# uc-vision/smart-tree

Measured on AMD Instinct MI355X. Metric: points/sec end-to-end (voxelize->sparse-UNet->skeleton), 1M-pt tree, higher is better.
Workload: dtype f32

## Files before the change

### smart_tree_amd/csrc/prims.hip

```cpp
#include <cstdarg>

#include "st_common.h"

static thread_local char g_err[512] = "";

void st_set_error(const char* fmt, ...) {
    va_list ap;
    va_start(ap, fmt);
    vsnprintf(g_err, sizeof(g_err), fmt, ap);
    va_end(ap);
}

extern "C" const char* st_last_error(void) { return g_err; }
void st_stream_wait(hipStream_t stream) { (void)hipStreamSynchronize(stream); }

extern "C" int st_version(void) { return 104; }

#define SCAN_BLOCK 256
#define SCAN_ITEMS 16
#define SCAN_TILE (SCAN_BLOCK * SCAN_ITEMS)
#define SCAN_DIRECT_BLOCKS 1024

__device__ __forceinline__ void scan_load(const uint32_t* in, int64_t base, int64_t n, uint32_t (&v)[SCAN_ITEMS]) {
    if (base + SCAN_ITEMS <= n && ((((uintptr_t)in) & 15) == 0)) {
        const uint4* p = reinterpret_cast<const uint4*>(in + base);
#pragma unroll
        for (int q = 0; q < SCAN_ITEMS / 4; q++) {
            const uint4 t = p[q];
            v[4 * q] = t.x; v[4 * q + 1] = t.y; v[4 * q + 2] = t.z; v[4 * q + 3] = t.w;
        }
    } else {
// ... 261 lines not shown
```

### smart_tree_amd/csrc/skeleton.hip

```cpp
#include "st_common.h"
#include "st_grid.h"
#include "smarttree_hip.h"

#include <atomic>

#define SK_MAX_WAVES 16
#define SK_EMPTY64 0xffffffffffffffffull
#define SK_WIDE_BLOCK 256
#define SK_SSSP_BLOCKS 2048
#define SK_MARK 0xfffffffeu
#define SK_ANC 64

struct SkJob {
    unsigned seq, done, quit;
    int len, id, csz, nrows, ny, x0, y0, z0, z1, path_off;
    float rp;
    unsigned gone;
    unsigned alive;
};

struct SkArgs {
    int C;
    int64_t m;
    const int* comp_off;
    const int* comp_seg;
    int* comp_of;
    const float* pts;
    const float* rad;
    const float* ysurf;
    const uint32_t* row_off;
    const uint32_t* col;
    const float* wgt;
    const StGrid* grid;
    const uint32_t* cell_start;
// ... 8 lines not shown
    int* n_branches;
    int* path_verts;
    int* branch_of;
    unsigned* dist_ord;
    unsigned* stamp;
    unsigned* q0;
    unsigned* q1;
    unsigned* term_bits;
    unsigned* help_bits;
    float4* pr;
    unsigned long long* best;
    unsigned* touched;
    int* anc;
    unsigned* cnt;
    unsigned* fcnt;
    unsigned fseg;
    int* s_done;
    int* s_len;
    int* s_cur_id;
    int* s_cur_off;
    int* s_nb;
    int* s_total;
    float* s_rp;
    unsigned* s_ntouched;
    int* s_cursor;
    int* s_wide;
    const unsigned* order;
    const float* order_init;
    const int* blk_comp;
    const int* blk_first;
// ... 40 lines not shown
__device__ __forceinline__ float sk_dist(const float* a, const float* b) {
    const float dx = a[0] - b[0], dy = a[1] - b[1], dz = a[2] - b[2];
    float s = dx * dx;
    float t = dy * dy;
    s = s + t;
    t = dz * dz;
    s = s + t;
    return s;
}

#define SK_VERTEX_LOOP(v) \
    for (int64_t v = (int64_t)blockIdx.x * blockDim.x + threadIdx.x; v < A.m; v += (int64_t)gridDim.x * blockDim.x)

#define SK_FS 16
#define SK_Q_HOLE 0xffffffffu
__device__ __forceinline__ unsigned sk_q_reserve(unsigned* q, unsigned* fc, unsigned seg, unsigned shard, unsigned n) {
    const unsigned at = atomicAdd(&fc[shard], n);
    if (at + n <= seg) return shard * seg + at;
    for (unsigned i = at; i < seg; i++) q[shard * seg + i] = SK_Q_HOLE;
    return SK_FS * seg + atomicAdd(&fc[SK_FS], n);
}

__device__ __forceinline__ unsigned sk_q_reserve_coop(unsigned* q, unsigned* fc, unsigned seg, unsigned shard, unsigned n) {
    const unsigned at = atomicAdd(&fc[shard], n);
    if (at + n <= seg) return shard * seg + at;
    for (unsigned i = at; i < seg; i++) __hip_atomic_store(&q[shard * seg + i], SK_Q_HOLE, __ATOMIC_RELAXED, __HIP_MEMORY_SCOPE_AGENT);
    return SK_FS * seg + atomicAdd(&fc[SK_FS], n);
}

__global__ void __launch_bounds__(SK_WIDE_BLOCK) k_sk_init(SkArgs A) {
    const unsigned inf = st_f2ord(__uint_as_float(0x7f800000u));
    SK_VERTEX_LOOP(v) { A.dist_ord[v] = inf; A.stamp[v] = 0u; }
    if (blockIdx.x == 0 && threadIdx.x < 8) A.cnt[threadIdx.x] = 0u;
    if (blockIdx.x == 0)
        for (int i = threadIdx.x; i < 3 * (SK_FS + 1); i += blockDim.x) A.fcnt[i] = i == SK_FS ? (unsigned)A.C : 0u;
}

__global__ void __launch_bounds__(1024) k_sk_roots(SkArgs A) {
    __shared__ unsigned long long s_red[SK_MAX_WAVES];
    const int c = blockIdx.x, base = A.comp_off[c], n = A.comp_off[c + 1] - base;
    unsigned long long key = 0;
    for (int v = threadIdx.x; v < n; v += blockDim.x) {
        A.comp_of[base + v] = c;
        const unsigned long long k = ((unsigned long long)(0xffffffffu - st_f2ord(A.ysurf[base + v])) << 32) | (0xffffffffu - (unsigned)v);
        key = k > key ? k : key;
    }
    key = block_max_u64(key, s_red);
    if (threadIdx.x == 0) {
// ... 38 lines not shown
    const unsigned round = (unsigned)r + 1u;
    const int lane = threadIdx.x & (glanes - 1);
    const unsigned wave = threadIdx.x / glanes, nwv = blockDim.x / glanes;
    const unsigned gw = blockIdx.x * nwv + wave, tw = gridDim.x * nwv;
#define SK_RELAX(u, du, out, out_n)                                                                        \
    {                                                                                                      \
        const uint32_t s_ = A.row_off[u], e_ = A.row_off[(u) + 1];                                         \
        for (uint32_t t = s_ + lane; t < e_; t += glanes) {                                                    \
            const unsigned v = A.col[t];                                                                   \
            const unsigned o = st_f2ord((du) + A.wgt[t]);                                                  \
            if (lookfirst && o >= A.dist_ord[v]) continue;  \
            const unsigned old = atomicMin(&A.dist_ord[v], o);                                             \
            if (o < old) {                                                                                 \
                const unsigned slot = atomicAdd(out_n, 1u);                                                \
                if (slot < SK_LQ) (out)[slot] = v;                                                         \
                else if (atomicExch(&A.stamp[v], round) != round) qn[sk_q_reserve(qn, fc_out, seg, shard, 1u)] = v; \
            }                                                                                              \
        }                                                                                                  \
    }
    for (unsigned f = gw; f < count; f += tw) {
        int sh = 0;
#pragma unroll
        for (int s_ = 1; s_ <= SK_FS; s_++) sh = f >= fpre[s_] ? s_ : sh;
        const unsigned u = q[(int64_t)sh * seg + (f - fpre[sh])];
        if (u == SK_Q_HOLE) continue;
        const float du = st_ord2f(A.dist_ord[u]);
        SK_RELAX(u, du, lq[0], &ln[0]);
    }
    int h = 1;
    for (; h < hops; h++) {
        __syncthreads();
        const unsigned have = ln[(h - 1) % 3];
        unsigned ncur = have < SK_LQ ? have : SK_LQ;
        if (ncur == 0) break;
        if (threadIdx.x == 0) ln[(h + 1) % 3] = 0;
        const unsigned* in = lq[(h - 1) & 1];
        unsigned* out = lq[h & 1];
        if (ncur > (unsigned)lcap) {
            for (unsigned i = lcap + threadIdx.x; i < ncur; i += blockDim.x) {
                const unsigned v = in[i];
                if (atomicExch(&A.stamp[v], round) != round) qn[sk_q_reserve(qn, fc_out, seg, shard, 1u)] = v;
            }
            ncur = (unsigned)lcap;
        }
        for (unsigned i = wave; i < ncur; i += nwv) {
            const unsigned u = in[i];
            const float du = st_ord2f(ld(&A.dist_ord[u]));
            SK_RELAX(u, du, out, &ln[h % 3]);
        }
    }
#undef SK_RELAX
    __syncthreads();
    const unsigned have = ln[(h - 1) % 3];
    const unsigned nrem = have < SK_LQ ? have : SK_LQ;
    const unsigned* rem = lq[(h - 1) & 1];
    unsigned* keep = lq[h & 1];
    unsigned* keep_n = &ln[h % 3];
    if (threadIdx.x == 0) *keep_n = 0;
    __syncthreads();
    for (unsigned i = threadIdx.x; i < nrem; i += blockDim.x) {
        const unsigned v = rem[i];
        if (atomicExch(&A.stamp[v], round) != round) keep[atomicAdd(keep_n, 1u)] = v;
    }
    __syncthreads();
    const unsigned nloc = *keep_n;
    if (threadIdx.x == 0 && nloc) lq_base = sk_q_reserve(qn, fc_out, seg, shard, nloc);
    __syncthreads();
    for (unsigned i = threadIdx.x; i < nloc; i += blockDim.x) qn[lq_base + i] = keep[i];
}


#define SK_COOP_BLOCKS 1024
#define SK_COOP_GROUP 32
#define SK_COOP_STRIDE 16
__device__ __forceinline__ unsigned ld_u(const unsigned* p) { return __hip_atomic_load(p, __ATOMIC_RELAXED, __HIP_MEMORY_SCOPE_AGENT); }
__device__ __forceinline__ void st_u(unsigned* p, unsigned v) { __hip_atomic_store(p, v, __ATOMIC_RELAXED, __HIP_MEMORY_SCOPE_AGENT); }

__device__ __forceinline__ bool sk_grid_barrier(unsigned* bar, unsigned round) {
    __shared__ int ok_;
    __syncthreads();
    if (threadIdx.x == 0) {
// ... 35 lines not shown
                const unsigned c_ = ld_u(&fc_in[s_]);
                run += s_ < SK_FS && c_ > seg ? seg : c_;
            }
            fpre[SK_FS + 1] = run;
        }
        if (threadIdx.x < 3) ln[threadIdx.x] = 0;
        __syncthreads();
        const unsigned count = fpre[SK_FS + 1];
        if (count == 0) {
            if (blockIdx.x == 0 && threadIdx.x == 0) st_u(&bar[2], (unsigned)r);
            return;
        }
        const unsigned* q = (r & 1) ? A.q1 : A.q0;
        unsigned* qn = (r & 1) ? A.q0 : A.q1;
        const unsigned round = (unsigned)r + 1u;
#define SK_QPUSH(v_) st_u(&qn[sk_q_reserve_coop(qn, fc_out, seg, shard, 1u)], (v_))
#define SK_RELAX_C(u, du, out, out_n)                                                                      \
    {                                                                                                      \
        const uint32_t s_ = A.row_off[u], e_ = A.row_off[(u) + 1];                                         \
        for (uint32_t t = s_ + lane; t < e_; t += glanes) {                                                \
            const unsigned v = A.col[t];                                                                   \
            const unsigned o = st_f2ord((du) + A.wgt[t]);                                                  \
            if (lookfirst && o >= ld_u(&A.dist_ord[v])) continue;                                          \
            const unsigned old = atomicMin(&A.dist_ord[v], o);                                             \
            if (o < old) {                                                                                 \
                const unsigned slot = atomicAdd(out_n, 1u);                                                \
                if (slot < SK_LQ) (out)[slot] = v;                                                         \
                else if (atomicExch(&A.stamp[v], round) != round) SK_QPUSH(v);                             \
            }                                                                                              \
        }                                                                                                  \
    }
// ... 31 lines not shown
#undef SK_RELAX_C
        __syncthreads();
        const unsigned have = ln[(h - 1) % 3];
        const unsigned nrem = have < SK_LQ ? have : SK_LQ;
        const unsigned* rem = lq[(h - 1) & 1];
        unsigned* keep = lq[h & 1];
        unsigned* keep_n = &ln[h % 3];
        if (threadIdx.x == 0) *keep_n = 0;
        __syncthreads();
        for (unsigned i = threadIdx.x; i < nrem; i += blockDim.x) {
            const unsigned v = rem[i];
            if (atomicExch(&A.stamp[v], round) != round) keep[atomicAdd(keep_n, 1u)] = v;
        }
        __syncthreads();
        const unsigned nloc = *keep_n;
        if (threadIdx.x == 0 && nloc) lq_base = sk_q_reserve_coop(qn, fc_out, seg, shard, nloc);
        __syncthreads();
        for (unsigned i = threadIdx.x; i < nloc; i += blockDim.x) st_u(&qn[lq_base + i], keep[i]);
#undef SK_QPUSH
        if (!sk_grid_barrier(bar, (unsigned)r)) return;
    }
}

__global__ void __launch_bounds__(SK_WIDE_BLOCK) k_sk_dist_out(SkArgs A) {
    SK_VERTEX_LOOP(v) A.dist[v] = st_ord2f(A.dist_ord[v]);
}

#define SK_PRED_LANES 8
__global__ void __launch_bounds__(SK_WIDE_BLOCK) k_sk_preds(SkArgs A) {
    const int sub = threadIdx.x & (SK_PRED_LANES - 1);
    const int64_t groups = ((int64_t)gridDim.x * blockDim.x) / SK_PRED_LANES;
    for (int64_t v = ((int64_t)blockIdx.x * blockDim.x + threadIdx.x) / SK_PRED_LANES; v < A.m; v += groups) {
        const int c = A.comp_of[v], base = A.comp_off[c];
        const bool is_root = (int)(v - base) == A.root_local[c];
        const float dv = A.dist[v];
        unsigned best = 0xffffffffu;
        if (!is_root)
            for (uint32_t t = A.row_off[v] + sub, e = A.row_off[v + 1]; t < e; t += SK_PRED_LANES) {
                const unsigned u = A.col[t];
                if (u == (unsigned)v) continue;
                const float du = A.dist[u];
                if (du < dv && du + A.wgt[t] == dv && u < best) best = u;
            }
        for (int d = SK_PRED_LANES / 2; d > 0; d >>= 1) { const unsigned o = __shfl_xor(best, d); best = o < best ? o : best; }
        if (sub != 0) continue;
        const bool ok = is_root || best != 0xffffffffu;
        A.pred[v] = (is_root || !ok) ? -1 : (int)best - base;
        A.stamp[v] = ok ? 1u : 0u;
        if (!ok) atomicAdd(&A.cnt[3], 1u);
    }
}

__global__ void __launch_bounds__(SK_WIDE_BLOCK) k_sk_preds_plateau(SkArgs A, unsigned round) {
    SK_VERTEX_LOOP(v) {
        if (A.stamp[v] != 0u) continue;
        const int base = A.comp_off[A.comp_of[v]];
        const float dv = A.dist[v];
        unsigned best = 0xffffffffu;
        for (uint32_t t = A.row_off[v]; t < A.row_off[v + 1]; t++) {
            const unsigned u = A.col[t];
            if (u == (unsigned)v) continue;
// ... 32 lines not shown
    const unsigned gw = (blockIdx.x * blockDim.x + threadIdx.x) >> 6, tw = (gridDim.x * blockDim.x) >> 6;
    for (unsigned f = gw; f < count; f += tw) {
        const unsigned u = q[f];
        const int base = A.comp_off[A.comp_of[u]];
        const float du = A.tree_dist[u];
        for (uint32_t t = A.row_off[u] + lane; t < A.row_off[u + 1]; t += 64) {
            const unsigned v = A.col[t];
            if (A.pred[v] != (int)u - base) continue;
            if (atomicExch(&A.stamp[v], SK_MARK) == SK_MARK) continue;
            A.tree_dist[v] = du + sqrtf(sk_dist(A.pts + 3 * (int64_t)v, A.pts + 3 * (int64_t)u));
            qn[atomicAdd(cnt_out, 1u)] = v;
        }
    }
}

__global__ void __launch_bounds__(SK_WIDE_BLOCK) k_sk_lift_init(SkArgs A) {
    SK_VERTEX_LOOP(v) {
        A.anc[v * SK_ANC] = A.pred[v];
        A.branch_of[v] = -1;
        A.best[v] = SK_EMPTY64;
        A.pr[v] = make_float4(A.pts[3 * v], A.pts[3 * v + 1], A.pts[3 * v + 2], A.rad[v]);
    }
    if (blockIdx.x == 0)
        for (int c = threadIdx.x; c < A.C; c += blockDim.x) { A.s_done[c] = 0; A.s_nb[c] = 0; A.s_total[c] = 0; A.s_len[c] = 0; A.s_cursor[c] = 0; A.s_wide[c] = 0; }
}

__device__ __forceinline__ float sk_initial_distance(const SkArgs& A, const float* distances, int64_t v) {
    return A.pred[v] > 0 ? distances[v] : -1.0f;
}

__global__ void __launch_bounds__(SK_WIDE_BLOCK) k_sk_sort_keys(SkArgs A, const float* distances, uint32_t* keys, uint32_t* vals, int pass) {
    SK_VERTEX_LOOP(v) {
        if (pass == 0) { keys[v] = ~st_f2ord(sk_initial_distance(A, distances, v)); vals[v] = (uint32_t)v; }
        else keys[v] = (uint32_t)A.comp_of[vals[v]];
    }
}

__global__ void __launch_bounds__(SK_WIDE_BLOCK) k_sk_order_init(SkArgs A, const float* distances, float* order_init) {
    SK_VERTEX_LOOP(j) order_init[j] = sk_initial_distance(A, distances, A.order[j]);
// ... 987 lines not shown
__global__ void k_sk_helper_tables(SkArgs A, int* hl_comp, int* hl_rank, int* c_nhelp) {
    if (blockIdx.x != 0 || threadIdx.x != 0) return;
    int at = 0;
    for (int c = 0; c < A.C; c++) {
        const int n = A.comp_off[c + 1] - A.comp_off[c];
        int k = n >= SK_HELP_MIN ? n / SK_HELP_PER : 0;
        k = k > SK_HELP_MAX ? SK_HELP_MAX : k;
        if (k > A.n_helpers - at) k = A.n_helpers - at;
        c_nhelp[c] = k;
        for (int j = 0; j < k; j++) { hl_comp[at] = c; hl_rank[at] = j + 1; at++; }
    }
    for (; at < A.n_helpers; at++) { hl_comp[at] = -1; hl_rank[at] = 0; }
}

#define SK_GRID_CELLS (1ll << 24)

struct SkLayout {
    unsigned *dist_ord, *stamp, *q0, *q1, *touched, *cnt, *s_ntouched, *sort_keys, *order, *coop_bar;
    float *s_rp, *order_init;
    unsigned* term_bits;
    float4* pr;
    int *s_cursor, *s_wide;
    char* sort_ws;
    int64_t sort_bytes;
    unsigned long long* best;
    int *anc, *comp_of, *s_done, *s_len, *s_cur_id, *s_cur_off, *s_nb, *s_total, *blk_comp, *blk_first, *blk_count, *hl_comp, *hl_rank, *c_nhelp;
    SkJob* jobs;
    StGrid* g;
    uint32_t* cell_start;
    float4* recs;
// ... 8 lines not shown
static inline int64_t sk_fseg(int64_t m, int64_t C) { return (m + C) / SK_FS > 0 ? (m + C) / SK_FS : 1; }
static inline int64_t sk_queue_words(int64_t m, int64_t C) { return SK_FS * sk_fseg(m, C) + (m + C); }
static inline int64_t sk_term_words(int64_t m, int64_t C) { return m / 32 + C + 2; }

static void sk_layout(StArena& a, int64_t m, int64_t C, SkLayout* s, int nseg = 1) {
    s->dist_ord = a.take<unsigned>(m);
    s->stamp = a.take<unsigned>(m);
    s->q0 = a.take<unsigned>(sk_queue_words(m, C));
    s->q1 = a.take<unsigned>(sk_queue_words(m, C));
    s->touched = a.take<unsigned>(m);
    s->term_bits = a.take<unsigned>(2 * sk_term_words(m, C));
    s->pr = a.take<float4>(m);
    s->best = a.take<unsigned long long>(m);
    s->anc = a.take<int>((int64_t)SK_ANC * m);
    s->comp_of = a.take<int>(m);
    s->cnt = a.take<unsigned>(8 + 3 * (SK_FS + 1));
    s->coop_bar = a.take<unsigned>(SK_COOP_STRIDE * (2 + SK_COOP_BLOCKS / SK_COOP_GROUP));
    s->s_done = a.take<int>(C);
    s->s_len = a.take<int>(C);
    s->s_cur_id = a.take<int>(C);
    s->s_cur_off = a.take<int>(C);
    s->s_nb = a.take<int>(C);
    s->s_total = a.take<int>(C);
    s->s_rp = a.take<float>(C);
    s->s_ntouched = a.take<unsigned>(C);
    s->s_cursor = a.take<int>(C);
    s->s_wide = a.take<int>(C);
    s->sort_keys = a.take<unsigned>(m);
    s->order = a.take<unsigned>(m);
    s->order_init = a.take<float>(m);
    s->sort_bytes = st_sort_ws_bytes(m);
// ... 7 lines not shown
    s->jobs = a.take<SkJob>(C);
    s->g = a.take<StGrid>(1);
    s->cell_start = a.take<uint32_t>(sk_grid_cells(nseg, m) + 1);
    s->recs = a.take<float4>(m);
    s->gws_bytes = st_grid_ws_bytes(m, sk_grid_cells(nseg, m));
    s->gws = a.take<char>(s->gws_bytes);
}

#define ST_TUNE_DEFAULT INT64_MIN
#define ST_TUNE_ENTRIES 24
#define SK_MAX_LAUNCH_BATCH 32
struct SkTuning {
    float prune_factor = 1.0f, grid_mean_mult = 1.0f;
    int small_work = SK_SMALL_WORK, iters_per_launch = SK_ITERS_PER_LAUNCH, launch_batch = 24, local_items = 0, wave_work = SK_WAVE_WORK, long_mode = 1;
    int sssp_hops = 6 , sssp_batch = 36 , sssp_lanes = 32, sssp_first = 2, sssp_blocks = SK_SSSP_BLOCKS, sssp_lcap = SK_LQ;
    int sssp_coop = 0, helpers = -1;
    long long help_lifetime_us = SK_HELP_LIFETIME_US, help_timeout_us = SK_HELP_TIMEOUT_US, help_announce_us = SK_HELP_ANNOUNCE_US;
    bool small_work_set = false, iters_set = false, long_set = false, launch_set = false;
    long long* ticks = nullptr;
    explicit SkTuning(const int64_t* t) {
        if (!t) return;
        auto has = [&](int i) { return t[i] != ST_TUNE_DEFAULT; };
        if (has(0)) prune_factor = (float)t[0] / 1000.0f;
        if (has(1)) { small_work = (int)t[1]; small_work_set = true; }
        if (has(2)) { iters_per_launch = (int)t[2]; iters_set = true; }
        if (has(3)) { launch_batch = t[3] < 1 ? 1 : (t[3] > SK_MAX_LAUNCH_BATCH ? SK_MAX_LAUNCH_BATCH : (int)t[3]); launch_set = true; }
        if (has(4)) local_items = (int)t[4];
        if (has(5)) wave_work = (int)t[5];
        if (has(6)) sssp_hops = t[6] < 1 ? 1 : (int)t[6];
        if (has(7)) sssp_batch = t[7] < 1 ? 1 : (t[7] > 64 ? 64 : (int)t[7]);
        if (has(8)) sssp_lanes = t[8] == 64 ? 64 : (t[8] == 32 ? 32 : 16);
        if (has(9)) sssp_first = t[9] < 1 ? 1 : (t[9] > 8 ? 8 : (int)t[9]);
        if (has(10)) sssp_blocks = t[10] < 1 ? 1 : (t[10] > 8192 ? 8192 : (int)t[10]);
        if (has(11)) grid_mean_mult = (float)t[11] / 100.0f;
        if (has(12)) { sssp_coop = (t[12] & 1) != 0; if (t[12] >= 256) helpers = (int)(t[12] >> 8) - 1; }
        if (has(13)) sssp_lcap = t[13] == 0 ? -SK_LQ : (t[13] > SK_LQ ? SK_LQ : (int)t[13]);
        if (has(14)) { long_mode = t[14] != 0; long_set = true; }
        if (has(15)) ticks = (long long*)(intptr_t)t[15];
        if (has(16)) help_lifetime_us = t[16] < 0 ? 0 : t[16];
        if (has(17)) help_timeout_us = t[17] < 0 ? 0 : t[17];
        if (has(18)) help_announce_us = t[18] < 0 ? 0 : t[18];
    }
};

static std::atomic<int> g_helpers_out{0};
static int sk_cu_count() {
    int dev = 0, cus = 0;
    if (hipGetDevice(&dev) != hipSuccess || hipDeviceGetAttribute(&cus, hipDeviceAttributeMultiprocessorCount, dev) != hipSuccess) {
        (void)hipGetLastError();
        return 0;
    }
    return cus;
}
static int sk_helper_cap() {
    const int cap = sk_cu_count() * 5 / 8;
    return cap < SK_HELP_POOL ? cap : SK_HELP_POOL;
}
struct SkHelperLease {
    int n = 0;
    int take(int want) {
        const int cap = sk_helper_cap();
        int cur = g_helpers_out.load();
        do { n = want < cap - cur ? want : cap - cur; if (n <= 0) { n = 0; return 0; } } while (!g_helpers_out.compare_exchange_weak(cur, cur + n));
        return n;
    }
    ~SkHelperLease() { if (n > 0) g_helpers_out.fetch_sub(n); }
};

static_assert(ST_TUNE_ENTRIES == ST_SKELETON_TUNING_ENTRIES, "header and library disagree about the tuning array");
extern "C" int st_abi_entries(int what) {
    return what == 0 ? ST_SKELETON_STATS_ENTRIES : (what == 1 ? ST_SKELETON_TUNING_ENTRIES : (what == 2 ? ST_MAX_SEG : -1));
}

extern "C" int64_t st_skeleton_workspace_bytes_seg(int64_t m, int64_t n_comp, int nseg) {
    StArena a(nullptr, 0);
    SkLayout s;
    sk_layout(a, m > 0 ? m : 1, n_comp > 0 ? n_comp : 1, &s, nseg);
    return a.used;
}
extern "C" int64_t st_skeleton_workspace_bytes(int64_t m, int64_t n_comp) { return st_skeleton_workspace_bytes_seg(m, n_comp, 1); }

// ... 32 lines not shown
    StArena a(ws, ws_bytes);
    SkLayout s;
    sk_layout(a, m, n_comp, &s, nseg);
    if (!a.ok() || !s.gws) {
        st_set_error("skeleton: workspace too small (%lld < %lld)", (long long)ws_bytes, (long long)a.used);
        return ST_ERR_WORKSPACE;
    }
    SkArgs A;
    memset(&A, 0, sizeof(A));
    A.C = n_comp; A.m = m; A.comp_off = comp_off; A.comp_seg = comp_seg; A.comp_of = s.comp_of; A.pts = pts; A.rad = rad; A.ysurf = ysurf;
    A.row_off = row_off; A.col = col; A.wgt = wgt; A.grid = s.g; A.cell_start = s.cell_start; A.recs = s.recs;
    A.dist = dist; A.pred = pred; A.root_local = root_local; A.tree_dist = tree_dist;
    A.branch_parent = branch_parent; A.branch_off = branch_off; A.branch_len = branch_len; A.n_branches = n_branches;
    A.path_verts = path_verts; A.branch_of = branch_of;
    A.dist_ord = s.dist_ord; A.stamp = s.stamp; A.q0 = s.q0; A.q1 = s.q1; A.term_bits = s.term_bits; A.help_bits = s.term_bits + sk_term_words(m, n_comp); A.pr = s.pr;
    A.best = s.best; A.touched = s.touched; A.anc = s.anc; A.cnt = s.cnt; A.fcnt = s.cnt + 8;
    A.fseg = (unsigned)sk_fseg(m, n_comp);
    A.s_done = s.s_done; A.s_len = s.s_len; A.s_cur_id = s.s_cur_id; A.s_cur_off = s.s_cur_off; A.s_nb = s.s_nb;
    A.s_total = s.s_total; A.s_rp = s.s_rp; A.s_ntouched = s.s_ntouched;
    A.blk_comp = s.blk_comp; A.blk_first = s.blk_first; A.blk_count = s.blk_count;
    A.s_cursor = s.s_cursor; A.s_wide = s.s_wide; A.order = s.order; A.order_init = s.order_init;
    A.hl_comp = s.hl_comp; A.hl_rank = s.hl_rank; A.c_nhelp = s.c_nhelp; A.jobs = s.jobs; A.n_helpers = 0;
    const SkTuning T(tuning);
    A.ticks = T.ticks;
    A.help_lifetime = T.help_lifetime_us * 100; A.help_timeout = T.help_timeout_us * 100; A.help_announce = T.help_announce_us * 100;
    A.prune_factor = T.prune_factor; A.small_work = T.small_work; A.iters_per_launch = T.iters_per_launch; A.local_items = T.local_items; A.wave_work = T.wave_work; A.long_mode = T.long_mode;
    int first_launches = T.launch_batch;
    SkHelperLease lease;
    int helpers_want = 0;
    if ((stages & 4) && T.helpers != 0 && block_threads >= 256 && m >= SK_HELP_MIN && (T.helpers > 0 || nseg <= SK_HELP_SEGS))
        helpers_want = T.helpers > 0 ? T.helpers : (int)st_min64(SK_HELP_POOL, m / SK_HELP_PER);
    const bool helpers_avail = lease.take(helpers_want) > 0;
    if (nseg > 1 || helpers_avail) {
        if (!T.small_work_set) A.small_work = 1 << 20;
        if (!T.iters_set) A.iters_per_launch = 1 << 20;
        if (!T.launch_set && A.long_mode && A.iters_per_launch >= (1 << 20)) first_launches = 1;
    } else if (!T.long_set) {
        A.long_mode = 0;
    }

    const unsigned vg = sk_vgrid(m);
    const unsigned fg = (unsigned)st_min64(st_div_up(m, SK_WIDE_BLOCK), T.sssp_blocks);
    unsigned h[8 + 3 * (SK_FS + 1)];
    int64_t sssp_rounds = 0;
    const bool defer_plateaus = (stages & 1) && (stages & 4) && !(stages & 2);
    auto resolve_plateaus = [&](unsigned unresolved) -> int {
        unsigned round = 2;
        while (unresolved > 0) {
            (void)hipMemsetAsync(&s.cnt[4], 0, sizeof(unsigned), stream);
            hipLaunchKernelGGL(k_sk_preds_plateau, dim3(vg), dim3(SK_WIDE_BLOCK), 0, stream, A, round);
            ST_TRY(sk_read(h, s.cnt, sizeof(unsigned) * 8, stream));
            if (h[4] == 0) break;
            unresolved -= h[4];
            round++;
        }
        if (stats_host) stats_host[1] = round - 2;
        return ST_OK;
    };
    auto run_sssp = [&]() -> int {
        hipLaunchKernelGGL(k_sk_init, dim3(vg), dim3(SK_WIDE_BLOCK), 0, stream, A);
        hipLaunchKernelGGL(k_sk_roots, dim3((unsigned)n_comp), dim3((unsigned)block_threads), 0, stream, A);
        bool coop_done = false;

        if (T.sssp_coop) {
            const int cus = sk_cu_count();
            const unsigned resident = cus > 1 ? (unsigned)st_min64(4ll * cus, SK_COOP_BLOCKS) : 1u;
            const unsigned cg = fg < resident ? fg : resident;
            (void)hipMemsetAsync(s.coop_bar, 0, SK_COOP_STRIDE * (2 + SK_COOP_BLOCKS / SK_COOP_GROUP) * sizeof(unsigned), stream);
            hipLaunchKernelGGL(k_sk_sssp_coop, dim3(cg), dim3(SK_WIDE_BLOCK), 0, stream, A, T.sssp_hops, T.sssp_lanes, T.sssp_lcap, s.coop_bar, 1 << 24);
            unsigned hb[4];
            ST_TRY(sk_read(hb, s.coop_bar, sizeof(hb), stream));
            if (hb[1] == 0u) { coop_done = true; sssp_rounds = hb[2]; }
            else {
                hipLaunchKernelGGL(k_sk_init, dim3(vg), dim3(SK_WIDE_BLOCK), 0, stream, A);
                hipLaunchKernelGGL(k_sk_roots, dim3((unsigned)n_comp), dim3((unsigned)block_threads), 0, stream, A);
            }
        }
        for (int r = 0; !coop_done;) {
            const int batch = r == 0 ? T.sssp_first * T.sssp_batch : T.sssp_batch;
            for (int b = 0; b < batch; b++, r++)
                hipLaunchKernelGGL(k_sk_sssp_round, dim3(fg), dim3(SK_WIDE_BLOCK), 0, stream, A, r, T.sssp_hops, T.sssp_lanes, T.sssp_lcap);
            ST_TRY(sk_read(h, s.cnt, sizeof(h), stream));
            sssp_rounds = r;
            unsigned left = 0;
            for (int i = 0; i <= SK_FS; i++) left |= h[8 + (r % 3) * (SK_FS + 1) + i];
            if (left == 0) break;
            ST_REQUIRE(r < (1 << 24), "skeleton: SSSP did not converge");
        }
        hipLaunchKernelGGL(k_sk_dist_out, dim3(vg), dim3(SK_WIDE_BLOCK), 0, stream, A);
        hipLaunchKernelGGL(k_sk_preds, dim3((unsigned)st_min64(st_div_up(m * SK_PRED_LANES, SK_WIDE_BLOCK), 8192)), dim3(SK_WIDE_BLOCK), 0, stream, A);
        if (stats_host) stats_host[0] = sssp_rounds;
        return ST_OK;
    };
    if (stages & 1) {
        ST_TRY(run_sssp());
        if (!defer_plateaus) {
            ST_TRY(sk_read(h, s.cnt, sizeof(unsigned) * 8, stream));
            ST_TRY(resolve_plateaus(h[3]));
        }
    }
    if (!(stages & 1)) hipLaunchKernelGGL(k_sk_fill_comp_of, dim3((unsigned)n_comp), dim3((unsigned)block_threads), 0, stream, A);
    if (stages & 2) {
        hipLaunchKernelGGL(k_sk_td_init, dim3(vg), dim3(SK_WIDE_BLOCK), 0, stream, A);
        hipLaunchKernelGGL(k_sk_td_roots, dim3(1), dim3(SK_WIDE_BLOCK), 0, stream, A);
        for (int r = 0;;) {
            for (int b = 0; b < 32; b++, r++)
                hipLaunchKernelGGL(k_sk_td_round, dim3(fg), dim3(SK_WIDE_BLOCK), 0, stream, A, r);
            ST_TRY(sk_read(h, s.cnt, sizeof(unsigned) * 8, stream));
            if (h[r % 3] == 0) break;
            ST_REQUIRE(r < (1 << 24), "skeleton: tree distance did not converge");
        }
    }
    if (stages & 4) {
        const int nblk = (int)st_min64((int64_t)n_comp + st_div_up(m, 1024), (int64_t)n_comp * SK_MAX_CLAIM_BLOCKS);
        hipLaunchKernelGGL(k_sk_blk_tables, dim3(1), dim3(1024), 0, stream, A, s.blk_comp, s.blk_first, s.blk_count, nblk);
        A.n_helpers = lease.n;
        hipLaunchKernelGGL(k_sk_helper_tables, dim3(1), dim3(64), 0, stream, A, s.hl_comp, s.hl_rank, s.c_nhelp);
        ST_TRY(st_grid_build(pts, m, grid_cell, sk_grid_cells(nseg, m), s.g, s.cell_start, s.recs, s.gws, s.gws_bytes, stream,
                             grid_cell < 0.0f ? -1.0f : 0.0f, grid_cell < 0.0f ? rad : nullptr, grid_cell < 0.0f ? m : 0,
                             vert_seg_off, nseg, vert_seg_off, T.grid_mean_mult));
        int64_t iters = 0;
        struct EventSet {
            hipEvent_t e[2 * SK_MAX_LAUNCH_BATCH];
            int n = 0;
            bool create() { for (; n < 2 * SK_MAX_LAUNCH_BATCH; n++) if (hipEventCreate(&e[n]) != hipSuccess) return false; return true; }
            ~EventSet() { for (int i = 0; i < n; i++) (void)hipEventDestroy(e[i]); }
        } evs;
        hipEvent_t* ev = evs.e;
        bool timing_ok = true;
        if (time_select && !evs.create()) { (void)hipGetLastError(); timing_ok = false; }
        const bool time_sel = time_select && timing_ok;
        double select_ms = 0.0;
        bool plateaus_pending = defer_plateaus;
        for (;;) {
            (void)hipMemsetAsync(&s.cnt[5], 0, 4 * sizeof(unsigned), stream);
            const float* distances = (stages & 2) ? tree_dist : dist;
            (void)hipMemsetAsync(s.term_bits, 0, 2 * sk_term_words(m, n_comp) * sizeof(unsigned), stream);
            hipLaunchKernelGGL(k_sk_lift_init, dim3(vg), dim3(SK_WIDE_BLOCK), 0, stream, A);
            for (int span = 1; span < SK_ANC; span *= 2)
                hipLaunchKernelGGL(k_sk_anc_pass, dim3(vg), dim3(SK_WIDE_BLOCK), 0, stream, A, span);
            hipLaunchKernelGGL(k_sk_sort_keys, dim3(vg), dim3(SK_WIDE_BLOCK), 0, stream, A, distances, s.sort_keys, s.order, 0);
            ST_TRY(st_radix_sort_pairs_u32(s.sort_keys, s.order, m, 32, s.sort_ws, s.sort_bytes, stream));
            if (n_comp > 1) {
                int bits = 1;
                while ((1ll << bits) < n_comp) bits++;
                hipLaunchKernelGGL(k_sk_sort_keys, dim3(vg), dim3(SK_WIDE_BLOCK), 0, stream, A, distances, s.sort_keys, s.order, 1);
                ST_TRY(st_radix_sort_pairs_u32(s.sort_keys, s.order, m, bits, s.sort_ws, s.sort_bytes, stream));
            }
            hipLaunchKernelGGL(k_sk_order_init, dim3(vg), dim3(SK_WIDE_BLOCK), 0, stream, A, distances, s.order_init);
            iters = 0;
            select_ms = 0.0;
            bool redo = false;
            for (int batch = first_launches;; batch = batch > 4 ? 4 : batch) {
                for (int b = 0; b < batch; b++, iters++) {
                    if (A.n_helpers > 0) (void)hipMemsetAsync(s.jobs, 0, (size_t)n_comp * sizeof(SkJob), stream);
                    if (time_sel) (void)hipEventRecord(ev[2 * b], stream);
                    hipLaunchKernelGGL(k_sk_select, dim3((unsigned)(A.n_helpers + n_comp)), dim3((unsigned)block_threads), 0, stream, A);
                    if (time_sel) (void)hipEventRecord(ev[2 * b + 1], stream);
                    hipLaunchKernelGGL(k_sk_claim, dim3((unsigned)nblk), dim3(SK_WIDE_BLOCK), 0, stream, A);
                }
                ST_TRY(sk_read(h, s.cnt, sizeof(unsigned) * 9, stream));
                if (time_sel)
                    for (int b = 0; b < batch; b++) {
                        float ms = 0.0f;
                        if (hipEventElapsedTime(&ms, ev[2 * b], ev[2 * b + 1]) == hipSuccess) select_ms += ms;
                        else { (void)hipGetLastError(); timing_ok = false; }
                    }
                if (plateaus_pending) {
                    plateaus_pending = false;
                    if (h[3] > 0) { redo = true; break; }
// ... 53 lines not shown
```

### smart_tree_amd/skeleton/skeletonize.py

```python
from __future__ import annotations

import ctypes
import os
from dataclasses import dataclass
from typing import List

import torch

from .. import _lib, profiling
from ..data_types.branch import BranchSkeleton
from ..data_types.cloud import Cloud
from ..data_types.tree import DisjointTreeSkeleton, TreeSkeleton
from .filter import outlier_removal
from . import tuning
from .graph import ComponentSet, medial_points, nn_graph

STAGE_SSSP, STAGE_TREE_DISTANCE, STAGE_SAMPLE = 1, 2, 4


GRID_DIV = 4.0


@dataclass
class ComponentResult:
# ... 55 lines not shown
        res.n_branches.zero_()
    stats = (ctypes.c_int64 * 16)()
    stats[7] = 1 if profiling.enabled() else 0
    nseg = comps.n_seg
    ws = _lib.workspace(L.st_skeleton_workspace_bytes_seg(m, C, nseg), dev)
    with profiling.stage("skeleton_kernels"):
        _lib.check(L.st_skeleton_components_seg(
            C, _lib.ptr(comps.comp_off.contiguous()), _lib.ptr(comps.comp_seg.contiguous()) if nseg > 1 else None,
            _lib.ptr(comps.vert_seg_off) if nseg > 1 else None, nseg, m, _lib.ptr(pts), _lib.ptr(rad), _lib.ptr(ys),
            _lib.ptr(comps.row_off), _lib.ptr(comps.col), _lib.ptr(comps.wgt), -float(GRID_DIV), int(stages),
            int(block_threads), _lib.ptr(res.dist), _lib.ptr(res.pred), _lib.ptr(res.root_local), _lib.ptr(res.tree_dist),
            _lib.ptr(res.branch_parent), _lib.ptr(res.branch_off), _lib.ptr(res.branch_len), _lib.ptr(res.n_branches),
            _lib.ptr(res.path_verts), _lib.ptr(res.branch_of), stats, _lib.ptr(ws), ws.numel(), _lib.stream(dev),
            tuning.skeleton_array()))
    res.stats = {"sssp_rounds": stats[0], "plateau_rounds": stats[1], "select_launches": stats[2], "lift_levels": stats[3],
                 "helpers_lost": int(stats[8]), "helpers": int(stats[9])}
    _note_helpers(res.stats)
    if stages & STAGE_SAMPLE:
        res.stats["branches"], res.stats["path_vertices"] = int(stats[6] & 0xFFFFFFFF), int(stats[6] >> 32)
    if stats[7] and stats[5]:
        claimed = (res.branch_of[:m] >= 0).sum()
        path_vertices = float(res.stats.get("path_vertices", 0))
        profiling.add_kernel_time("k_sk_select", stats[4] * 1e-6, stats[5],
                                  lambda: path_vertices * 24.0 + float(claimed.item()) * 16.0 + m * 8.0,
                                  chip_share=comps.n_components / float(profiling.compute_units(dev)))
    return res


class Skeletonizer:
    def __init__(self, K: int, min_connection_length: float, minimum_graph_vertices: int,
                 device: torch.device = torch.device("cuda:0")):
# ... 301 lines not shown
```

### smart_tree_amd/skeleton/tuning.py

```python
from __future__ import annotations

import contextlib
import ctypes
import os
import threading

DEFAULT = -(1 << 63)
KNN_CELL_MEAN_MULT = 100
TICKS = 15
HELP_LIFETIME_US, HELP_TIMEOUT_US, HELP_ANNOUNCE_US = 16, 17, 18
ENTRIES = 24

_local = threading.local()


def _env_defaults() -> dict:
    out = {}
    for kv in filter(None, os.environ.get("ST_SKELETON_PARAMS", "").split(",")):
        which, value = kv.split("=")
        out[int(which)] = int(value)
    return out


_ENV = _env_defaults()

# ... 37 lines not shown
```

Baseline: 901.5 million.

## Overlap skeleton selection prep and sorting with ancestor passes on a side stream

Adds a pooled side stream with events and moves selection preparation (block tables, helper tables, grid build, term-bit clear, point/radius packing) onto it, forking and joining around the main stream. By default this runs after SSSP, and with overlap=2 it runs during SSSP. The distance sort and order_init also run on the side stream while the ancestor-lifting passes run on the main stream. The change also folds the dist_out kernel into k_sk_preds, moves per-pass memsets into k_sk_lift_init, skips redundant first-iteration memsets, and adds an SSSP queue-overflow counter. It risks extra event and stream overhead and new cross-stream hazards on shared buffers.

```diff
diff --git a/smart_tree_amd/csrc/prims.hip b/smart_tree_amd/csrc/prims.hip
--- a/smart_tree_amd/csrc/prims.hip
+++ b/smart_tree_amd/csrc/prims.hip
@@ -14,7 +14,7 @@
 extern "C" const char* st_last_error(void) { return g_err; }
 void st_stream_wait(hipStream_t stream) { (void)hipStreamSynchronize(stream); }
 
-extern "C" int st_version(void) { return 104; }
+extern "C" int st_version(void) { return 105; }
 
 #define SCAN_BLOCK 256
 #define SCAN_ITEMS 16
diff --git a/smart_tree_amd/csrc/skeleton.hip b/smart_tree_amd/csrc/skeleton.hip
--- a/smart_tree_amd/csrc/skeleton.hip
+++ b/smart_tree_amd/csrc/skeleton.hip
@@ -3,6 +3,8 @@
 #include "smarttree_hip.h"
 
 #include <atomic>
+#include <mutex>
+#include <vector>
 
 #define SK_MAX_WAVES 16
 #define SK_EMPTY64 0xffffffffffffffffull
@@ -18,6 +20,8 @@
     unsigned gone;
     unsigned alive;
 };
+
+static_assert(sizeof(SkJob) % sizeof(unsigned) == 0, "k_sk_lift_init clears the job records word by word");
 
 struct SkArgs {
     int C;
@@ -56,6 +60,7 @@
     int* anc;
     unsigned* cnt;
     unsigned* fcnt;
+    unsigned* fovf;
     unsigned fseg;
     int* s_done;
     int* s_len;
@@ -126,16 +131,18 @@
 
 #define SK_FS 16
 #define SK_Q_HOLE 0xffffffffu
-__device__ __forceinline__ unsigned sk_q_reserve(unsigned* q, unsigned* fc, unsigned seg, unsigned shard, unsigned n) {
+__device__ __forceinline__ unsigned sk_q_reserve(unsigned* q, unsigned* fc, unsigned seg, unsigned shard, unsigned n, unsigned* ovf) {
     const unsigned at = atomicAdd(&fc[shard], n);
     if (at + n <= seg) return shard * seg + at;
+    atomicAdd(ovf, 1u);
     for (unsigned i = at; i < seg; i++) q[shard * seg + i] = SK_Q_HOLE;
     return SK_FS * seg + atomicAdd(&fc[SK_FS], n);
 }
 
-__device__ __forceinline__ unsigned sk_q_reserve_coop(unsigned* q, unsigned* fc, unsigned seg, unsigned shard, unsigned n) {
+__device__ __forceinline__ unsigned sk_q_reserve_coop(unsigned* q, unsigned* fc, unsigned seg, unsigned shard, unsigned n, unsigned* ovf) {
     const unsigned at = atomicAdd(&fc[shard], n);
     if (at + n <= seg) return shard * seg + at;
+    atomicAdd(ovf, 1u);
     for (unsigned i = at; i < seg; i++) __hip_atomic_store(&q[shard * seg + i], SK_Q_HOLE, __ATOMIC_RELAXED, __HIP_MEMORY_SCOPE_AGENT);
     return SK_FS * seg + atomicAdd(&fc[SK_FS], n);
 }
@@ -144,6 +151,7 @@
     const unsigned inf = st_f2ord(__uint_as_float(0x7f800000u));
     SK_VERTEX_LOOP(v) { A.dist_ord[v] = inf; A.stamp[v] = 0u; }
     if (blockIdx.x == 0 && threadIdx.x < 8) A.cnt[threadIdx.x] = 0u;
+    if (blockIdx.x == 0 && threadIdx.x == 8) *A.fovf = 0u;
     if (blockIdx.x == 0)
         for (int i = threadIdx.x; i < 3 * (SK_FS + 1); i += blockDim.x) A.fcnt[i] = i == SK_FS ? (unsigned)A.C : 0u;
 }
@@ -212,7 +220,7 @@
             if (o < old) {                                                                                 \
                 const unsigned slot = atomicAdd(out_n, 1u);                                                \
                 if (slot < SK_LQ) (out)[slot] = v;                                                         \
-                else if (atomicExch(&A.stamp[v], round) != round) qn[sk_q_reserve(qn, fc_out, seg, shard, 1u)] = v; \
+                else if (atomicExch(&A.stamp[v], round) != round) qn[sk_q_reserve(qn, fc_out, seg, shard, 1u, A.fovf)] = v; \
             }                                                                                              \
         }                                                                                                  \
     }
@@ -237,7 +245,7 @@
         if (ncur > (unsigned)lcap) {
             for (unsigned i = lcap + threadIdx.x; i < ncur; i += blockDim.x) {
                 const unsigned v = in[i];
-                if (atomicExch(&A.stamp[v], round) != round) qn[sk_q_reserve(qn, fc_out, seg, shard, 1u)] = v;
+                if (atomicExch(&A.stamp[v], round) != round) qn[sk_q_reserve(qn, fc_out, seg, shard, 1u, A.fovf)] = v;
             }
             ncur = (unsigned)lcap;
         }
@@ -262,7 +270,7 @@
     }
     __syncthreads();
     const unsigned nloc = *keep_n;
-    if (threadIdx.x == 0 && nloc) lq_base = sk_q_reserve(qn, fc_out, seg, shard, nloc);
+    if (threadIdx.x == 0 && nloc) lq_base = sk_q_reserve(qn, fc_out, seg, shard, nloc, A.fovf);
     __syncthreads();
     for (unsigned i = threadIdx.x; i < nloc; i += blockDim.x) qn[lq_base + i] = keep[i];
 }
@@ -328,7 +336,7 @@
         const unsigned* q = (r & 1) ? A.q1 : A.q0;
         unsigned* qn = (r & 1) ? A.q0 : A.q1;
         const unsigned round = (unsigned)r + 1u;
-#define SK_QPUSH(v_) st_u(&qn[sk_q_reserve_coop(qn, fc_out, seg, shard, 1u)], (v_))
+#define SK_QPUSH(v_) st_u(&qn[sk_q_reserve_coop(qn, fc_out, seg, shard, 1u, &bar[3])], (v_))
 #define SK_RELAX_C(u, du, out, out_n)                                                                      \
     {                                                                                                      \
         const uint32_t s_ = A.row_off[u], e_ = A.row_off[(u) + 1];                                         \
@@ -390,16 +398,12 @@
         }
         __syncthreads();
         const unsigned nloc = *keep_n;
-        if (threadIdx.x == 0 && nloc) lq_base = sk_q_reserve_coop(qn, fc_out, seg, shard, nloc);
+        if (threadIdx.x == 0 && nloc) lq_base = sk_q_reserve_coop(qn, fc_out, seg, shard, nloc, &bar[3]);
         __syncthreads();
         for (unsigned i = threadIdx.x; i < nloc; i += blockDim.x) st_u(&qn[lq_base + i], keep[i]);
 #undef SK_QPUSH
         if (!sk_grid_barrier(bar, (unsigned)r)) return;
     }
-}
-
-__global__ void __launch_bounds__(SK_WIDE_BLOCK) k_sk_dist_out(SkArgs A) {
-    SK_VERTEX_LOOP(v) A.dist[v] = st_ord2f(A.dist_ord[v]);
 }
 
 #define SK_PRED_LANES 8
@@ -409,18 +413,19 @@
     for (int64_t v = ((int64_t)blockIdx.x * blockDim.x + threadIdx.x) / SK_PRED_LANES; v < A.m; v += groups) {
         const int c = A.comp_of[v], base = A.comp_off[c];
         const bool is_root = (int)(v - base) == A.root_local[c];
-        const float dv = A.dist[v];
+        const float dv = st_ord2f(A.dist_ord[v]);
         unsigned best = 0xffffffffu;
         if (!is_root)
             for (uint32_t t = A.row_off[v] + sub, e = A.row_off[v + 1]; t < e; t += SK_PRED_LANES) {
                 const unsigned u = A.col[t];
                 if (u == (unsigned)v) continue;
-                const float du = A.dist[u];
+                const float du = st_ord2f(A.dist_ord[u]);
                 if (du < dv && du + A.wgt[t] == dv && u < best) best = u;
             }
         for (int d = SK_PRED_LANES / 2; d > 0; d >>= 1) { const unsigned o = __shfl_xor(best, d); best = o < best ? o : best; }
         if (sub != 0) continue;
         const bool ok = is_root || best != 0xffffffffu;
+        A.dist[v] = dv;
         A.pred[v] = (is_root || !ok) ? -1 : (int)best - base;
         A.stamp[v] = ok ? 1u : 0u;
         if (!ok) atomicAdd(&A.cnt[3], 1u);
@@ -483,15 +488,25 @@
     }
 }
 
+__global__ void __launch_bounds__(SK_WIDE_BLOCK) k_sk_pr_init(SkArgs A) {
+    SK_VERTEX_LOOP(v) A.pr[v] = make_float4(A.pts[3 * v], A.pts[3 * v + 1], A.pts[3 * v + 2], A.rad[v]);
+}
+
 __global__ void __launch_bounds__(SK_WIDE_BLOCK) k_sk_lift_init(SkArgs A) {
     SK_VERTEX_LOOP(v) {
         A.anc[v * SK_ANC] = A.pred[v];
         A.branch_of[v] = -1;
         A.best[v] = SK_EMPTY64;
-        A.pr[v] = make_float4(A.pts[3 * v], A.pts[3 * v + 1], A.pts[3 * v + 2], A.rad[v]);
-    }
-    if (blockIdx.x == 0)
+    }
+    if (blockIdx.x == 0) {
         for (int c = threadIdx.x; c < A.C; c += blockDim.x) { A.s_done[c] = 0; A.s_nb[c] = 0; A.s_total[c] = 0; A.s_len[c] = 0; A.s_cursor[c] = 0; A.s_wide[c] = 0; }
+        if (threadIdx.x < 4) A.cnt[5 + threadIdx.x] = 0u;
+    }
+    if (A.n_helpers > 0) {
+        unsigned* jw = (unsigned*)A.jobs;
+        const int64_t words = (int64_t)A.C * (int64_t)(sizeof(SkJob) / sizeof(unsigned));
+        for (int64_t i = (int64_t)blockIdx.x * blockDim.x + threadIdx.x; i < words; i += (int64_t)gridDim.x * blockDim.x) jw[i] = 0u;
+    }
 }
 
 __device__ __forceinline__ float sk_initial_distance(const SkArgs& A, const float* distances, int64_t v) {
@@ -1509,6 +1524,7 @@
 }
 
 #define SK_GRID_CELLS (1ll << 24)
+#define SK_CNT_WORDS (8 + 3 * (SK_FS + 1) + 1)
 
 struct SkLayout {
     unsigned *dist_ord, *stamp, *q0, *q1, *touched, *cnt, *s_ntouched, *sort_keys, *order, *coop_bar;
@@ -1547,7 +1563,7 @@
     s->best = a.take<unsigned long long>(m);
     s->anc = a.take<int>((int64_t)SK_ANC * m);
     s->comp_of = a.take<int>(m);
-    s->cnt = a.take<unsigned>(8 + 3 * (SK_FS + 1));
+    s->cnt = a.take<unsigned>(SK_CNT_WORDS);
     s->coop_bar = a.take<unsigned>(SK_COOP_STRIDE * (2 + SK_COOP_BLOCKS / SK_COOP_GROUP));
     s->s_done = a.take<int>(C);
     s->s_len = a.take<int>(C);
@@ -1585,6 +1601,7 @@
     float prune_factor = 1.0f, grid_mean_mult = 1.0f;
     int small_work = SK_SMALL_WORK, iters_per_launch = SK_ITERS_PER_LAUNCH, launch_batch = 24, local_items = 0, wave_work = SK_WAVE_WORK, long_mode = 1;
     int sssp_hops = 6 , sssp_batch = 36 , sssp_lanes = 32, sssp_first = 2, sssp_blocks = SK_SSSP_BLOCKS, sssp_lcap = SK_LQ;
+    int overlap = 1;
     int sssp_coop = 0, helpers = -1;
     long long help_lifetime_us = SK_HELP_LIFETIME_US, help_timeout_us = SK_HELP_TIMEOUT_US, help_announce_us = SK_HELP_ANNOUNCE_US;
     bool small_work_set = false, iters_set = false, long_set = false, launch_set = false;
@@ -1611,6 +1628,7 @@
         if (has(16)) help_lifetime_us = t[16] < 0 ? 0 : t[16];
         if (has(17)) help_timeout_us = t[17] < 0 ? 0 : t[17];
         if (has(18)) help_announce_us = t[18] < 0 ? 0 : t[18];
+        if (has(19)) overlap = t[19] < 0 ? 0 : (t[19] > 2 ? 2 : (int)t[19]);
     }
 };
 
@@ -1636,6 +1654,73 @@
         return n;
     }
     ~SkHelperLease() { if (n > 0) g_helpers_out.fetch_sub(n); }
+};
+
+struct SkSide {
+    int dev = 0;
+    hipStream_t stream = nullptr;
+    hipEvent_t ev[4];
+};
+static std::mutex g_side_mu;
+static std::vector<SkSide*> g_side_free;
+struct SkSideLease {
+    SkSide* s = nullptr;
+    hipStream_t main = nullptr;
+    bool open = false;
+    int take(hipStream_t main_) {
+        main = main_;
+#ifdef ST_HIPEMU
+        static SkSide emu;
+        s = &emu;
+        s->stream = main_;
+        return ST_OK;
+#else
+        int dev = 0;
+        if (hipGetDevice(&dev) != hipSuccess) { (void)hipGetLastError(); st_set_error("skeleton: no current device"); return ST_ERR_LAUNCH; }
+        {
+            std::lock_guard<std::mutex> g(g_side_mu);
+            for (size_t i = 0; i < g_side_free.size(); i++)
+                if (g_side_free[i]->dev == dev) { s = g_side_free[i]; g_side_free.erase(g_side_free.begin() + (long)i); return ST_OK; }
+        }
+        SkSide* n = new SkSide;
+        n->dev = dev;
+        bool ok = hipStreamCreateWithFlags(&n->stream, hipStreamNonBlocking) == hipSuccess;
+        for (int i = 0; ok && i < 4; i++) ok = hipEventCreateWithFlags(&n->ev[i], hipEventDisableTiming) == hipSuccess;
+        if (!ok) {
+            st_set_error("skeleton: cannot create the side stream: %s", hipGetErrorString(hipGetLastError()));
+            return ST_ERR_LAUNCH;
+        }
+        s = n;
+        return ST_OK;
+#endif
+    }
+    hipStream_t stream() const { return s->stream; }
+    void fork(int e) {
+        open = true;
+#ifndef ST_HIPEMU
+        (void)hipEventRecord(s->ev[e], main);
+        (void)hipStreamWaitEvent(s->stream, s->ev[e], 0);
+#else
+        (void)e;
+#endif
+    }
+    void join(int e) {
+        open = false;
+#ifndef ST_HIPEMU
+        (void)hipEventRecord(s->ev[e], s->stream);
+        (void)hipStreamWaitEvent(main, s->ev[e], 0);
+#else
+        (void)e;
+#endif
+    }
+    ~SkSideLease() {
+        if (!s) return;
+        if (open) join(3);
+#ifndef ST_HIPEMU
+        std::lock_guard<std::mutex> g(g_side_mu);
+        g_side_free.push_back(s);
+#endif
+    }
 };
 
 static_assert(ST_TUNE_ENTRIES == ST_SKELETON_TUNING_ENTRIES, "header and library disagree about the tuning array");
@@ -1698,7 +1783,7 @@
     A.branch_parent = branch_parent; A.branch_off = branch_off; A.branch_len = branch_len; A.n_branches = n_branches;
     A.path_verts = path_verts; A.branch_of = branch_of;
     A.dist_ord = s.dist_ord; A.stamp = s.stamp; A.q0 = s.q0; A.q1 = s.q1; A.term_bits = s.term_bits; A.help_bits = s.term_bits + sk_term_words(m, n_comp); A.pr = s.pr;
-    A.best = s.best; A.touched = s.touched; A.anc = s.anc; A.cnt = s.cnt; A.fcnt = s.cnt + 8;
+    A.best = s.best; A.touched = s.touched; A.anc = s.anc; A.cnt = s.cnt; A.fcnt = s.cnt + 8; A.fovf = s.cnt + SK_CNT_WORDS - 1;
     A.fseg = (unsigned)sk_fseg(m, n_comp);
     A.s_done = s.s_done; A.s_len = s.s_len; A.s_cur_id = s.s_cur_id; A.s_cur_off = s.s_cur_off; A.s_nb = s.s_nb;
     A.s_total = s.s_total; A.s_rp = s.s_rp; A.s_ntouched = s.s_ntouched;
@@ -1725,8 +1810,27 @@
 
     const unsigned vg = sk_vgrid(m);
     const unsigned fg = (unsigned)st_min64(st_div_up(m, SK_WIDE_BLOCK), T.sssp_blocks);
-    unsigned h[8 + 3 * (SK_FS + 1)];
-    int64_t sssp_rounds = 0;
+    const int nblk = (int)st_min64((int64_t)n_comp + st_div_up(m, 1024), (int64_t)n_comp * SK_MAX_CLAIM_BLOCKS);
+    const int overlap = (stages & 4) ? T.overlap : 0;
+    SkSideLease side;
+    if (overlap) ST_TRY(side.take(stream));
+    A.n_helpers = (stages & 4) ? lease.n : 0;
+    auto prepare_selection = [&](hipStream_t st) -> int {
+        hipLaunchKernelGGL(k_sk_blk_tables, dim3(1), dim3(1024), 0, st, A, s.blk_comp, s.blk_first, s.blk_count, nblk);
+        hipLaunchKernelGGL(k_sk_helper_tables, dim3(1), dim3(64), 0, st, A, s.hl_comp, s.hl_rank, s.c_nhelp);
+        ST_TRY(st_grid_build(pts, m, grid_cell, sk_grid_cells(nseg, m), s.g, s.cell_start, s.recs, s.gws, s.gws_bytes, st,
+                             grid_cell < 0.0f ? -1.0f : 0.0f, grid_cell < 0.0f ? rad : nullptr, grid_cell < 0.0f ? m : 0,
+                             vert_seg_off, nseg, vert_seg_off, T.grid_mean_mult));
+        (void)hipMemsetAsync(s.term_bits, 0, 2 * sk_term_words(m, n_comp) * sizeof(unsigned), st);
+        hipLaunchKernelGGL(k_sk_pr_init, dim3(vg), dim3(SK_WIDE_BLOCK), 0, st, A);
+        return ST_OK;
+    };
+    if (overlap == 2) {
+        side.fork(0);
+        ST_TRY(prepare_selection(side.stream()));
+    }
+    unsigned h[SK_CNT_WORDS];
+    int64_t sssp_rounds = 0, sssp_overflows = 0;
     const bool defer_plateaus = (stages & 1) && (stages & 4) && !(stages & 2);
     auto resolve_plateaus = [&](unsigned unresolved) -> int {
         unsigned round = 2;
@@ -1754,7 +1858,7 @@
             hipLaunchKernelGGL(k_sk_sssp_coop, dim3(cg), dim3(SK_WIDE_BLOCK), 0, stream, A, T.sssp_hops, T.sssp_lanes, T.sssp_lcap, s.coop_bar, 1 << 24);
             unsigned hb[4];
             ST_TRY(sk_read(hb, s.coop_bar, sizeof(hb), stream));
-            if (hb[1] == 0u) { coop_done = true; sssp_rounds = hb[2]; }
+            if (hb[1] == 0u) { coop_done = true; sssp_rounds = hb[2]; sssp_overflows = hb[3]; }
             else {
                 hipLaunchKernelGGL(k_sk_init, dim3(vg), dim3(SK_WIDE_BLOCK), 0, stream, A);
                 hipLaunchKernelGGL(k_sk_roots, dim3((unsigned)n_comp), dim3((unsigned)block_threads), 0, stream, A);
@@ -1766,14 +1870,14 @@
                 hipLaunchKernelGGL(k_sk_sssp_round, dim3(fg), dim3(SK_WIDE_BLOCK), 0, stream, A, r, T.sssp_hops, T.sssp_lanes, T.sssp_lcap);
             ST_TRY(sk_read(h, s.cnt, sizeof(h), stream));
             sssp_rounds = r;
+            sssp_overflows = h[SK_CNT_WORDS - 1];
             unsigned left = 0;
             for (int i = 0; i <= SK_FS; i++) left |= h[8 + (r % 3) * (SK_FS + 1) + i];
             if (left == 0) break;
             ST_REQUIRE(r < (1 << 24), "skeleton: SSSP did not converge");
         }
-        hipLaunchKernelGGL(k_sk_dist_out, dim3(vg), dim3(SK_WIDE_BLOCK), 0, stream, A);
         hipLaunchKernelGGL(k_sk_preds, dim3((unsigned)st_min64(st_div_up(m * SK_PRED_LANES, SK_WIDE_BLOCK), 8192)), dim3(SK_WIDE_BLOCK), 0, stream, A);
-        if (stats_host) stats_host[0] = sssp_rounds;
+        if (stats_host) { stats_host[0] = sssp_rounds; stats_host[10] = sssp_overflows; }
         return ST_OK;
     };
     if (stages & 1) {
@@ -1796,13 +1900,12 @@
         }
     }
     if (stages & 4) {
-        const int nblk = (int)st_min64((int64_t)n_comp + st_div_up(m, 1024), (int64_t)n_comp * SK_MAX_CLAIM_BLOCKS);
-        hipLaunchKernelGGL(k_sk_blk_tables, dim3(1), dim3(1024), 0, stream, A, s.blk_comp, s.blk_first, s.blk_count, nblk);
-        A.n_helpers = lease.n;
-        hipLaunchKernelGGL(k_sk_helper_tables, dim3(1), dim3(64), 0, stream, A, s.hl_comp, s.hl_rank, s.c_nhelp);
-        ST_TRY(st_grid_build(pts, m, grid_cell, sk_grid_cells(nseg, m), s.g, s.cell_start, s.recs, s.gws, s.gws_bytes, stream,
-                             grid_cell < 0.0f ? -1.0f : 0.0f, grid_cell < 0.0f ? rad : nullptr, grid_cell < 0.0f ? m : 0,
-                             vert_seg_off, nseg, vert_seg_off, T.grid_mean_mult));
+        if (overlap == 1) {
+            side.fork(0);
+            ST_TRY(prepare_selection(side.stream()));
+        } else if (!overlap) {
+            ST_TRY(prepare_selection(stream));
+        }
         int64_t iters = 0;
         struct EventSet {
             hipEvent_t e[2 * SK_MAX_LAUNCH_BATCH];
@@ -1816,28 +1919,35 @@
         const bool time_sel = time_select && timing_ok;
         double select_ms = 0.0;
         bool plateaus_pending = defer_plateaus;
-        for (;;) {
-            (void)hipMemsetAsync(&s.cnt[5], 0, 4 * sizeof(unsigned), stream);
+        for (int pass = 0;; pass++) {
             const float* distances = (stages & 2) ? tree_dist : dist;
-            (void)hipMemsetAsync(s.term_bits, 0, 2 * sk_term_words(m, n_comp) * sizeof(unsigned), stream);
+            if (pass > 0) (void)hipMemsetAsync(s.term_bits, 0, 2 * sk_term_words(m, n_comp) * sizeof(unsigned), stream);
+            const hipStream_t so = overlap ? side.stream() : stream;
+            if (overlap) side.fork(2);
             hipLaunchKernelGGL(k_sk_lift_init, dim3(vg), dim3(SK_WIDE_BLOCK), 0, stream, A);
-            for (int span = 1; span < SK_ANC; span *= 2)
-                hipLaunchKernelGGL(k_sk_anc_pass, dim3(vg), dim3(SK_WIDE_BLOCK), 0, stream, A, span);
-            hipLaunchKernelGGL(k_sk_sort_keys, dim3(vg), dim3(SK_WIDE_BLOCK), 0, stream, A, distances, s.sort_keys, s.order, 0);
-            ST_TRY(st_radix_sort_pairs_u32(s.sort_keys, s.order, m, 32, s.sort_ws, s.sort_bytes, stream));
+            if (!overlap)
+                for (int span = 1; span < SK_ANC; span *= 2)
+                    hipLaunchKernelGGL(k_sk_anc_pass, dim3(vg), dim3(SK_WIDE_BLOCK), 0, stream, A, span);
+            hipLaunchKernelGGL(k_sk_sort_keys, dim3(vg), dim3(SK_WIDE_BLOCK), 0, so, A, distances, s.sort_keys, s.order, 0);
+            ST_TRY(st_radix_sort_pairs_u32(s.sort_keys, s.order, m, 32, s.sort_ws, s.sort_bytes, so));
             if (n_comp > 1) {
                 int bits = 1;
                 while ((1ll << bits) < n_comp) bits++;
-                hipLaunchKernelGGL(k_sk_sort_keys, dim3(vg), dim3(SK_WIDE_BLOCK), 0, stream, A, distances, s.sort_keys, s.order, 1);
-                ST_TRY(st_radix_sort_pairs_u32(s.sort_keys, s.order, m, bits, s.sort_ws, s.sort_bytes, stream));
-            }
-            hipLaunchKernelGGL(k_sk_order_init, dim3(vg), dim3(SK_WIDE_BLOCK), 0, stream, A, distances, s.order_init);
+                hipLaunchKernelGGL(k_sk_sort_keys, dim3(vg), dim3(SK_WIDE_BLOCK), 0, so, A, distances, s.sort_keys, s.order, 1);
+                ST_TRY(st_radix_sort_pairs_u32(s.sort_keys, s.order, m, bits, s.sort_ws, s.sort_bytes, so));
+            }
+            hipLaunchKernelGGL(k_sk_order_init, dim3(vg), dim3(SK_WIDE_BLOCK), 0, so, A, distances, s.order_init);
+            if (overlap) {
+                for (int span = 1; span < SK_ANC; span *= 2)
+                    hipLaunchKernelGGL(k_sk_anc_pass, dim3(vg), dim3(SK_WIDE_BLOCK), 0, stream, A, span);
+                side.join(3);
+            }
             iters = 0;
             select_ms = 0.0;
             bool redo = false;
             for (int batch = first_launches;; batch = batch > 4 ? 4 : batch) {
                 for (int b = 0; b < batch; b++, iters++) {
-                    if (A.n_helpers > 0) (void)hipMemsetAsync(s.jobs, 0, (size_t)n_comp * sizeof(SkJob), stream);
+                    if (A.n_helpers > 0 && iters > 0) (void)hipMemsetAsync(s.jobs, 0, (size_t)n_comp * sizeof(SkJob), stream);
                     if (time_sel) (void)hipEventRecord(ev[2 * b], stream);
                     hipLaunchKernelGGL(k_sk_select, dim3((unsigned)(A.n_helpers + n_comp)), dim3((unsigned)block_threads), 0, stream, A);
                     if (time_sel) (void)hipEventRecord(ev[2 * b + 1], stream);
diff --git a/smart_tree_amd/skeleton/skeletonize.py b/smart_tree_amd/skeleton/skeletonize.py
--- a/smart_tree_amd/skeleton/skeletonize.py
+++ b/smart_tree_amd/skeleton/skeletonize.py
@@ -93,7 +93,7 @@
             _lib.ptr(res.path_verts), _lib.ptr(res.branch_of), stats, _lib.ptr(ws), ws.numel(), _lib.stream(dev),
             tuning.skeleton_array()))
     res.stats = {"sssp_rounds": stats[0], "plateau_rounds": stats[1], "select_launches": stats[2], "lift_levels": stats[3],
-                 "helpers_lost": int(stats[8]), "helpers": int(stats[9])}
+                 "helpers_lost": int(stats[8]), "helpers": int(stats[9]), "sssp_overflows": int(stats[10])}
     _note_helpers(res.stats)
     if stages & STAGE_SAMPLE:
         res.stats["branches"], res.stats["path_vertices"] = int(stats[6] & 0xFFFFFFFF), int(stats[6] >> 32)
diff --git a/smart_tree_amd/skeleton/tuning.py b/smart_tree_amd/skeleton/tuning.py
--- a/smart_tree_amd/skeleton/tuning.py
+++ b/smart_tree_amd/skeleton/tuning.py
@@ -9,6 +9,7 @@
 KNN_CELL_MEAN_MULT = 100
 TICKS = 15
 HELP_LIFETIME_US, HELP_TIMEOUT_US, HELP_ANNOUNCE_US = 16, 17, 18
+OVERLAP = 19
 ENTRIES = 24
 
 _local = threading.local()
```

Measured after the change: 885.2 million. 1.8% lower.
